# youssefg7/dl-sound-classification

Hardware: AMD Instinct MI355X
Metric: training clips/sec (EnvNet-v2, ESC-50 shape) (higher is better)
Workload: dtype bf16; 1 GPU; EnvNet-v2 train step (BC-mix, fwd, soft-CE, bwd, clip, Adam), ESC-50 shape; global_batch=256, per_gpu_batch=256, clip_samples=220500, parallelism=dp1, model=envnet_v2

## Files before the change

### dl-sound-classification_amd/csrc/gemm_common.h

```cpp
#pragma once
#include "common.h"
#include "optim_update.h"

namespace mgemm {

struct EpiDev {
  char* ptr;
  int dtype, act, accumulate, aux_dtype;
  int64_t ldc, rm_inner, rm_outer, rm_istride, rm_offset;
  const float* bias;
  const char* aux;
  int64_t ldaux;
  float alpha, act_scale;
  double* sqsum;
};

template <class R>
struct UpdateEpi {
  float* p;
  float* s0;
  float* s1;
  bf16* shadow;
  const float* coef;
  int64_t ld;
  int first;
  R rule;
};

struct DArgs {
  const bf16* a;
  const bf16* b;
  int64_t lda, ldb, M, N, K, kper;
  int split, nbm, nbn;
  int nfast;
  int gm;
  float* ws;
  EpiDev e;
  int mode;
  UpdateEpi<mopt::AdamRule> upd;
};

static __device__ __forceinline__ void epi_store(const EpiDev& e, int64_t m, int64_t n, float acc) {
  float v = acc * e.alpha;
  if (e.bias) v += e.bias[n];
  switch (e.act) {
    case MIA_ACT_RELU: v = fmaxf(v, 0.f); break;
    case MIA_ACT_GELU: v = gelu_erf(v); break;
    case MIA_DACT_NZ: {
      const float a = ld_elem(e.aux, e.aux_dtype, m * e.ldaux + n);
      v = a != 0.f ? v * e.act_scale : 0.f;
      break;
    }
    case MIA_DACT_GELU: v *= gelu_erf_grad(ld_elem(e.aux, e.aux_dtype, m * e.ldaux + n)); break;
    case MIA_ACT_ADD_AUX: v += ld_elem(e.aux, e.aux_dtype, m * e.ldaux + n); break;
    case MIA_ACT_GELU_SAVE:
      st_elem(const_cast<char*>(e.aux), e.aux_dtype, m * e.ldaux + n, v);
      v = gelu_erf(v);
      break;
    case MIA_ACT_GELU_SAVE_D:
      st_elem(const_cast<char*>(e.aux), e.aux_dtype, m * e.ldaux + n, gelu_erf_grad(v));
      v = gelu_erf(v);
      break;
    case MIA_DACT_MUL: v *= ld_elem(e.aux, e.aux_dtype, m * e.ldaux + n); break;
    default: break;
  }
  int64_t prow = m;
  if (e.rm_inner) {
    if (e.rm_offset == MIA_RM_DROP) {
      const int64_t x = m % e.rm_inner;
      if (x >= e.rm_outer) return;
      prow = (m / e.rm_inner) * e.rm_outer + x;
    } else {
      prow = (m / e.rm_inner) * e.rm_outer + (m % e.rm_inner) * e.rm_istride + e.rm_offset;
    }
  }
  const int64_t idx = prow * e.ldc + n;
  if (e.accumulate) v += ld_elem(e.ptr, e.dtype, idx);
  st_elem(e.ptr, e.dtype, idx, v);
}

static __device__ __forceinline__ void ld16(const void* p, int dtype, int64_t idx, float* f) {
  if (dtype == MIA_BF16) {
    const uint4* q = reinterpret_cast<const uint4*>(reinterpret_cast<const bf16*>(p) + idx);
#pragma unroll
    for (int h = 0; h < 2; ++h) {
      const uint4 u = q[h];
      const uint32_t w[4] = {u.x, u.y, u.z, u.w};
#pragma unroll
      for (int i = 0; i < 4; ++i) {
        f[8 * h + 2 * i] = __uint_as_float(w[i] << 16);
        f[8 * h + 2 * i + 1] = __uint_as_float(w[i] & 0xffff0000u);
      }
    }
  } else {
    const float4* q = reinterpret_cast<const float4*>(reinterpret_cast<const float*>(p) + idx);
#pragma unroll
    for (int h = 0; h < 4; ++h) {
      const float4 u = q[h];
      f[4 * h] = u.x; f[4 * h + 1] = u.y; f[4 * h + 2] = u.z; f[4 * h + 3] = u.w;
    }
  }
}

static __device__ __forceinline__ void st16(void* p, int dtype, int64_t idx, const float* o) {
  if (dtype == MIA_BF16) {
    uint32_t w[8];
#pragma unroll
    for (int c = 0; c < 8; ++c) {
      w[c] = pk_bf16(o[2 * c], o[2 * c + 1]);
    }
    uint4* d = reinterpret_cast<uint4*>(reinterpret_cast<bf16*>(p) + idx);
    d[0] = make_uint4(w[0], w[1], w[2], w[3]);
    d[1] = make_uint4(w[4], w[5], w[6], w[7]);
  } else {
    float4* d = reinterpret_cast<float4*>(reinterpret_cast<float*>(p) + idx);
#pragma unroll
    for (int q = 0; q < 4; ++q) d[q] = make_float4(o[4 * q], o[4 * q + 1], o[4 * q + 2], o[4 * q + 3]);
  }
}

static __device__ __forceinline__ void epi_store16(const EpiDev& e, int64_t m, int64_t n0, int64_t N, const float* v) {
  int64_t prow = m;
  if (e.rm_inner) {
    if (e.rm_offset == MIA_RM_DROP) {
      const int64_t x = m % e.rm_inner;
      if (x >= e.rm_outer) return;
      prow = (m / e.rm_inner) * e.rm_outer + x;
    } else {
      prow = (m / e.rm_inner) * e.rm_outer + (m % e.rm_inner) * e.rm_istride + e.rm_offset;
    }
  }
  const int64_t idx = prow * e.ldc + n0;
  const bool uses_aux = e.act == MIA_DACT_NZ || e.act == MIA_DACT_GELU || e.act == MIA_ACT_ADD_AUX ||
                        e.act == MIA_ACT_GELU_SAVE || e.act == MIA_ACT_GELU_SAVE_D || e.act == MIA_DACT_MUL;
  const int64_t aidx = m * e.ldaux + n0;
  const bool fast = n0 + 16 <= N && !e.accumulate &&
                    ((idx * (e.dtype == MIA_BF16 ? 2 : 4)) & 15) == 0 &&
                    ((reinterpret_cast<uintptr_t>(e.ptr)) & 15) == 0 &&
                    (!uses_aux || (((aidx * (e.aux_dtype == MIA_BF16 ? 2 : 4)) & 15) == 0 &&
                                   ((reinterpret_cast<uintptr_t>(e.aux)) & 15) == 0));
  if (!fast) {
    for (int c = 0; c < 16; ++c)
      if (n0 + c < N) epi_store(e, m, n0 + c, v[c]);
    return;
  }
  float o[16];
#pragma unroll
  for (int c = 0; c < 16; ++c) o[c] = v[c] * e.alpha;
  if (e.bias) {
    const float4* b4 = reinterpret_cast<const float4*>(e.bias + n0);
    const bool ba = ((reinterpret_cast<uintptr_t>(e.bias + n0)) & 15) == 0;
#pragma unroll
    for (int q = 0; q < 4; ++q) {
      float4 bb;
      if (ba) bb = b4[q];
      else bb = make_float4(e.bias[n0 + 4 * q], e.bias[n0 + 4 * q + 1], e.bias[n0 + 4 * q + 2], e.bias[n0 + 4 * q + 3]);
      o[4 * q] += bb.x; o[4 * q + 1] += bb.y; o[4 * q + 2] += bb.z; o[4 * q + 3] += bb.w;
    }
  }
  if (e.act == MIA_ACT_RELU) {
#pragma unroll
    for (int c = 0; c < 16; ++c) o[c] = fmaxf(o[c], 0.f);
  } else if (e.act == MIA_ACT_GELU) {
#pragma unroll
    for (int c = 0; c < 16; ++c) o[c] = gelu_erf(o[c]);
  } else if (e.act == MIA_ACT_GELU_SAVE) {
    st16(const_cast<char*>(e.aux), e.aux_dtype, aidx, o);
#pragma unroll
    for (int c = 0; c < 16; ++c) o[c] = gelu_erf(o[c]);
  } else if (e.act == MIA_ACT_GELU_SAVE_D) {
    float d[16];
#pragma unroll
    for (int c = 0; c < 16; ++c) d[c] = gelu_erf_grad(o[c]);
    st16(const_cast<char*>(e.aux), e.aux_dtype, aidx, d);
#pragma unroll
    for (int c = 0; c < 16; ++c) o[c] = gelu_erf(o[c]);
  } else if (uses_aux) {
    float a[16];
    ld16(e.aux, e.aux_dtype, aidx, a);
    if (e.act == MIA_DACT_NZ) {
#pragma unroll
      for (int c = 0; c < 16; ++c) o[c] = a[c] != 0.f ? o[c] * e.act_scale : 0.f;
    } else if (e.act == MIA_DACT_GELU) {
#pragma unroll
      for (int c = 0; c < 16; ++c) o[c] *= gelu_erf_grad(a[c]);
    } else if (e.act == MIA_DACT_MUL) {
#pragma unroll
      for (int c = 0; c < 16; ++c) o[c] *= a[c];
    } else {
#pragma unroll
      for (int c = 0; c < 16; ++c) o[c] += a[c];
    }
  }
  st16(e.ptr, e.dtype, idx, o);
}


EpiDev to_dev(const MiaEpilogue& e);
void launch_splitk_reduce(const float* ws, int split, int64_t M, int64_t N, const EpiDev& e, hipStream_t s);

int igemm_run(const MiaOperand& A, const MiaOperand& B, const MiaEpilogue& E, int64_t M, int64_t N, int64_t K,
              int compute, int split, void* workspace, hipStream_t s);
bool rowconv_ok(const MiaOperand& A, const MiaOperand& B, int64_t M, int64_t N, int64_t K, int compute, int split);
int rowconv_run(const MiaOperand& A, const MiaOperand& B, const MiaEpilogue& E, int64_t M, int64_t N, hipStream_t s);
bool rowwgrad_ok(const MiaOperand& A, const MiaOperand& B, int64_t M, int64_t N, int64_t K, int compute, int split);
int rowwgrad_run(const MiaOperand& A, const MiaOperand& B, const MiaEpilogue& E, int64_t M, int64_t N, int split,
                 void* workspace, hipStream_t s);
bool wgrad8_ok(const MiaOperand& A, const MiaOperand& B, int64_t M);
int wgrad8_run(const MiaOperand& A, const MiaOperand& B, const MiaEpilogue& E, int64_t M, int64_t N, int split,
               void* workspace, hipStream_t s);
bool tapwgrad_ok(const MiaOperand& A, const MiaOperand& B, int64_t M, int64_t N, int64_t K, int compute, int split);
int tapwgrad_run(const MiaOperand& A, const MiaOperand& B, const MiaEpilogue& E, int64_t M, int64_t N, int split,
                 void* workspace, hipStream_t s);
bool tapconv_ok(const MiaOperand& A, const MiaOperand& B, int64_t M, int64_t N, int64_t K, int compute, int split);
int tapconv_run(const MiaOperand& A, const MiaOperand& B, const MiaEpilogue& E, hipStream_t s);
bool dgemm_ok(const MiaOperand& A, const MiaOperand& B, int64_t M, int64_t N, int64_t K, int compute);
int dgemm_run(const MiaOperand& A, const MiaOperand& B, const MiaEpilogue& E, int64_t M, int64_t N, int64_t K,
              int split, void* workspace, hipStream_t s);
int tile_sqsum_run(const float* c, int64_t ldc, int64_t M, int64_t N, double* sqsum, hipStream_t s);
bool mg_ok(const MiaOperand& A, const MiaOperand& B, const MiaEpilogue& E, int64_t M, int64_t N, int64_t K,
           int compute);
int mg_split(int64_t M, int64_t N, int64_t K);
int64_t mg_workspace_bytes(int64_t M, int64_t N, int64_t K, int colsum, int a_colsum = 0);
int mg_run(const MiaOperand& A, const MiaOperand& B, const MiaEpilogue& E, int64_t M, int64_t N, int64_t K,
           void* workspace, hipStream_t s);


}
```

### dl-sound-classification_amd/csrc/wgrad8.hip

```cpp
#include "gemm_common.h"

namespace mgemm {

struct W8Args {
  const bf16* x;
  const bf16* dy;
  const float* ps;
  const float* pt;
  int n, h, w, oh, ow;
  int nblk;
  float* ws;
};

namespace {

constexpr int W8_NT = 512;
constexpr int W8_BP = 128;
constexpr int W8_WPX = W8_BP + 7;
constexpr int W8_XROW = W8_WPX * 64;
constexpr int W8_RING = 9;
constexpr int W8_DROW = W8_BP * 64;
constexpr int W8_XCH = (W8_WPX * 4 + W8_NT - 1) / W8_NT;

typedef short s16x8 __attribute__((ext_vector_type(8)));
typedef unsigned u32x4 __attribute__((ext_vector_type(4)));

__device__ __forceinline__ bf16x8 tr_frag(const char* p0, int stride) {
  const s16x4 lo = __builtin_amdgcn_ds_read_tr16_b64_v4i16((MIA_LDS s16x4*)(p0));
  const s16x4 hi = __builtin_amdgcn_ds_read_tr16_b64_v4i16((MIA_LDS s16x4*)(p0 + 4 * stride));
  const s16x8 c = {lo[0], lo[1], lo[2], lo[3], hi[0], hi[1], hi[2], hi[3]};
  return __builtin_bit_cast(bf16x8, c);
}

__device__ __forceinline__ u32x4 bn_relu_pack(u32x4 u, bool ok, const float* sc, const float* sh) {
  if (!ok) return u32x4{0u, 0u, 0u, 0u};
  uint32_t w4[4];
#pragma unroll
  for (int i = 0; i < 4; ++i) {
    const float lo = fmaxf(fmaf(__uint_as_float(u[i] << 16), sc[2 * i], sh[2 * i]), 0.f);
    const float hi = fmaxf(fmaf(__uint_as_float(u[i] & 0xffff0000u), sc[2 * i + 1], sh[2 * i + 1]), 0.f);
    w4[i] = pk_bf16(lo, hi);
  }
  return u32x4{w4[0], w4[1], w4[2], w4[3]};
}

__global__ __launch_bounds__(W8_NT) void wgrad8_kernel(W8Args g) {
  __shared__ __attribute__((aligned(16))) char smem[W8_RING * W8_XROW + 2 * W8_DROW];
  char* ring = smem;
  char* dys = smem + W8_RING * W8_XROW;
  const int t = threadIdx.x, lane = t & 63;
  const int ky = __builtin_amdgcn_readfirstlane(t >> 6);
  const int i16 = lane & 15, gq = lane >> 4;
  const int cg = t & 3;
  float sc[8], sh[8];
#pragma unroll
  for (int i = 0; i < 8; ++i) { sc[i] = g.ps[cg * 8 + i]; sh[i] = g.pt[cg * 8 + i]; }

  f32x16 acc[8];
#pragma unroll
  for (int q = 0; q < 8; ++q)
#pragma unroll
    for (int r = 0; r < 16; ++r) acc[q][r] = 0.f;

  const int nchunk = (g.ow + W8_BP - 1) / W8_BP;
  const int items = g.n * nchunk;
  u32x4 xr[W8_XCH], dr;
  uint32_t xok = 0;
  bool dok = false;
  const u32x4* xs = reinterpret_cast<const u32x4*>(g.x);
  const u32x4* ds = reinterpret_cast<const u32x4*>(g.dy);

  for (int item = blockIdx.x; item < items; item += gridDim.x) {
    const int b = item / nchunk;
    const int x0 = (item - b * nchunk) * W8_BP;
    auto load_x = [&](int iy) __attribute__((always_inline)) {
      xok = 0;
#pragma unroll
      for (int i = 0; i < W8_XCH; ++i) {
        const int q = t + W8_NT * i;
        const int px = x0 + (q >> 2);
        const bool ok = (q >> 2) < W8_WPX && px < g.w && iy < g.h;
        const int64_t off = ok ? ((((int64_t)b * g.h + iy) * g.w + px) * 4 + (q & 3)) : 0;
        xr[i] = xs[off];
        xok |= (uint32_t)ok << i;
      }
    };
    auto load_dy = [&](int oy) __attribute__((always_inline)) {
      const int px = x0 + (t >> 2);
      dok = oy >= 0 && oy < g.oh && px < g.ow;
      const int64_t off = dok ? ((((int64_t)b * g.oh + oy) * g.ow + px) * 4 + (t & 3)) : 0;
      dr = ds[off];
    };
    auto store_x = [&](int slot) __attribute__((always_inline)) {
#pragma unroll
      for (int i = 0; i < W8_XCH; ++i) {
        const int q = t + W8_NT * i;
        if ((q >> 2) < W8_WPX)
          *reinterpret_cast<u32x4*>(ring + slot * W8_XROW + q * 16) = bn_relu_pack(xr[i], (xok >> i) & 1u, sc, sh);
      }
    };
    auto store_dy = [&](int buf) __attribute__((always_inline)) {
      *reinterpret_cast<u32x4*>(dys + buf * W8_DROW + t * 16) = dok ? dr : u32x4{0u, 0u, 0u, 0u};
    };

    load_x(0);
    store_x(0);
    __syncthreads();
    for (int s = 0; s < g.h; ++s) {
      load_x(s + 1);
      load_dy(s - 6);
      const int oy = s - 7;
      if (oy >= 0) {
        const char* xrow = ring + ((oy + ky) % W8_RING) * W8_XROW;
        const char* drow = dys + (oy & 1) * W8_DROW;
#pragma unroll
        for (int ks = 0; ks < W8_BP / 16; ++ks) {
          const int kr = ks * 16 + 8 * (gq >> 1) + (i16 >> 2);
          const int c4 = 16 * (gq & 1) + 4 * (i16 & 3);
          const bf16x8 fa = tr_frag(drow + kr * 64 + c4 * 2, 64);
#pragma unroll
          for (int kx = 0; kx < 8; ++kx) {
            const bf16x8 fb = tr_frag(xrow + (kr + kx) * 64 + c4 * 2, 64);
            acc[kx] = __builtin_amdgcn_mfma_f32_32x32x16_bf16(fa, fb, acc[kx], 0, 0, 0);
          }
        }
      }
      if (s + 1 < g.h) store_x((s + 1) % W8_RING);
      if (s - 6 >= 0 && s - 6 < g.oh) store_dy((s - 6) & 1);
      __syncthreads();
    }
  }

  float* dst = g.ws + (int64_t)blockIdx.x * 32 * 2048 + ky * 256;
#pragma unroll
  for (int kx = 0; kx < 8; ++kx)
#pragma unroll
    for (int r = 0; r < 16; ++r) {
      const int co = (r & 3) + 8 * (r >> 2) + 4 * (lane >> 5);
      dst[(int64_t)co * 2048 + kx * 32 + (lane & 31)] = acc[kx][r];
    }
}

}

bool wgrad8_ok(const MiaOperand& A, const MiaOperand& B, int64_t M) {
  return A.dtype == MIA_BF16 && M == 32 && B.c == 32 && B.kh == 8 && B.kw == 8 && B.sw == 1 && B.ph == 0 &&
         B.pw == 0 && B.pre == MIA_PRE_AFFINE_RELU && B.h == B.oh + 7 && B.w == B.ow + 7;
}

int wgrad8_run(const MiaOperand& A, const MiaOperand& B, const MiaEpilogue& E, int64_t M, int64_t N, int split,
               void* workspace, hipStream_t s) {
  W8Args w8;
  w8.x = reinterpret_cast<const bf16*>(B.ptr);
  w8.dy = reinterpret_cast<const bf16*>(A.ptr);
  w8.ps = B.pre_scale; w8.pt = B.pre_shift;
  w8.n = B.n; w8.h = B.h; w8.w = B.w; w8.oh = B.oh; w8.ow = B.ow;
  const int64_t items = (int64_t)B.n * cdiv(B.ow, 128);
  w8.nblk = (int)std::min<int64_t>(std::min<int64_t>(split, 256), items);
  w8.ws = reinterpret_cast<float*>(workspace);
  wgrad8_kernel<<<w8.nblk, W8_NT, 0, s>>>(w8);
  hipError_t err = hipGetLastError();
  if (err != hipSuccess) return mia::fail(-(int)err, "wgrad8 launch: %s", hipGetErrorString(err));
  launch_splitk_reduce(w8.ws, w8.nblk, M, N, to_dev(E), s);
  MIA_LAUNCH_CHECK("splitk_reduce");
  return 0;
}

}
```

Before: 15510 clips/s.

## Pipeline wgrad8 kernel: shared transposed runs, interleaved staging, tail k-step skip

Reworks the 8x8 weight-gradient conv kernel. Each k-step now loads one transposed LDS run and derives all eight kx-shifted B fragments by register alignbit, replacing eight separate transposed reads. A and B fragments are double-buffered across k-steps, and the global loads and LDS stores for the next row are spread across specific k-steps with sched_group_barrier hints so they overlap the MFMAs. The kernel also preloads the first rows in batches and skips k-steps past the output width. The old path stays selectable through the MIA_WGRAD_V1 environment variable. The cost is more scheduling complexity and register pressure.

```diff
diff --git a/dl-sound-classification_amd/csrc/gemm_common.h b/dl-sound-classification_amd/csrc/gemm_common.h
--- a/dl-sound-classification_amd/csrc/gemm_common.h
+++ b/dl-sound-classification_amd/csrc/gemm_common.h
@@ -1,4 +1,6 @@
 #pragma once
+#include <cstdlib>
+
 #include "common.h"
 #include "optim_update.h"
 
@@ -195,6 +197,46 @@
   st16(e.ptr, e.dtype, idx, o);
 }
 
+
+static __device__ __forceinline__ bf16x8 tr_frag(const char* p0, int stride) {
+  typedef short s16x8_ __attribute__((ext_vector_type(8)));
+  const s16x4 lo = __builtin_amdgcn_ds_read_tr16_b64_v4i16((MIA_LDS s16x4*)(p0));
+  const s16x4 hi = __builtin_amdgcn_ds_read_tr16_b64_v4i16((MIA_LDS s16x4*)(p0 + 4 * stride));
+  const s16x8_ c = {lo[0], lo[1], lo[2], lo[3], hi[0], hi[1], hi[2], hi[3]};
+  return __builtin_bit_cast(bf16x8, c);
+}
+
+template <int G>
+struct TrRun {
+  uint32_t d[2 * G];
+};
+template <int G>
+static __device__ __forceinline__ TrRun<G> tr_run(const char* p0, int stride) {
+  typedef uint32_t u32x2_ __attribute__((ext_vector_type(2)));
+  TrRun<G> r;
+#pragma unroll
+  for (int q = 0; q < G; ++q) {
+    const u32x2_ v = __builtin_bit_cast(
+        u32x2_, __builtin_amdgcn_ds_read_tr16_b64_v4i16((MIA_LDS s16x4*)(p0 + 4 * q * stride)));
+    r.d[2 * q] = v[0];
+    r.d[2 * q + 1] = v[1];
+  }
+  return r;
+}
+template <int KX, int G>
+static __device__ __forceinline__ bf16x8 shifted_frag(const TrRun<G>& r) {
+  typedef uint32_t u32x4_ __attribute__((ext_vector_type(4)));
+  static_assert(KX >= 0 && (KX + 1) / 2 + 3 < 2 * G, "shift past the run");
+  u32x4_ o;
+#pragma unroll
+  for (int i = 0; i < 4; ++i) {
+    if constexpr (KX % 2 == 0) o[i] = r.d[KX / 2 + i];
+    else o[i] = __builtin_amdgcn_alignbit(r.d[KX / 2 + i + 1], r.d[KX / 2 + i], 16);
+  }
+  return __builtin_bit_cast(bf16x8, o);
+}
+
+static inline bool wgrad_v1() { const char* e = getenv("MIA_WGRAD_V1"); return e && e[0] == '1'; }
 
 EpiDev to_dev(const MiaEpilogue& e);
 void launch_splitk_reduce(const float* ws, int split, int64_t M, int64_t N, const EpiDev& e, hipStream_t s);
diff --git a/dl-sound-classification_amd/csrc/wgrad8.hip b/dl-sound-classification_amd/csrc/wgrad8.hip
--- a/dl-sound-classification_amd/csrc/wgrad8.hip
+++ b/dl-sound-classification_amd/csrc/wgrad8.hip
@@ -21,15 +21,20 @@
 constexpr int W8_RING = 9;
 constexpr int W8_DROW = W8_BP * 64;
 constexpr int W8_XCH = (W8_WPX * 4 + W8_NT - 1) / W8_NT;
-
-typedef short s16x8 __attribute__((ext_vector_type(8)));
+constexpr int W8_STAGE_KS = 5;
+static_assert(W8_XCH == 2 && W8_BP * 4 == W8_NT && W8_STAGE_KS + 2 < W8_BP / 16, "staging is spread over three k-steps");
+
 typedef unsigned u32x4 __attribute__((ext_vector_type(4)));
 
-__device__ __forceinline__ bf16x8 tr_frag(const char* p0, int stride) {
-  const s16x4 lo = __builtin_amdgcn_ds_read_tr16_b64_v4i16((MIA_LDS s16x4*)(p0));
-  const s16x4 hi = __builtin_amdgcn_ds_read_tr16_b64_v4i16((MIA_LDS s16x4*)(p0 + 4 * stride));
-  const s16x8 c = {lo[0], lo[1], lo[2], lo[3], hi[0], hi[1], hi[2], hi[3]};
-  return __builtin_bit_cast(bf16x8, c);
+__device__ __forceinline__ void mfma_taps(f32x16 (&acc)[8], bf16x8 fa, const TrRun<4>& run) {
+  acc[0] = __builtin_amdgcn_mfma_f32_32x32x16_bf16(fa, shifted_frag<0>(run), acc[0], 0, 0, 0);
+  acc[1] = __builtin_amdgcn_mfma_f32_32x32x16_bf16(fa, shifted_frag<1>(run), acc[1], 0, 0, 0);
+  acc[2] = __builtin_amdgcn_mfma_f32_32x32x16_bf16(fa, shifted_frag<2>(run), acc[2], 0, 0, 0);
+  acc[3] = __builtin_amdgcn_mfma_f32_32x32x16_bf16(fa, shifted_frag<3>(run), acc[3], 0, 0, 0);
+  acc[4] = __builtin_amdgcn_mfma_f32_32x32x16_bf16(fa, shifted_frag<4>(run), acc[4], 0, 0, 0);
+  acc[5] = __builtin_amdgcn_mfma_f32_32x32x16_bf16(fa, shifted_frag<5>(run), acc[5], 0, 0, 0);
+  acc[6] = __builtin_amdgcn_mfma_f32_32x32x16_bf16(fa, shifted_frag<6>(run), acc[6], 0, 0, 0);
+  acc[7] = __builtin_amdgcn_mfma_f32_32x32x16_bf16(fa, shifted_frag<7>(run), acc[7], 0, 0, 0);
 }
 
 __device__ __forceinline__ u32x4 bn_relu_pack(u32x4 u, bool ok, const float* sc, const float* sh) {
@@ -44,6 +49,18 @@
   return u32x4{w4[0], w4[1], w4[2], w4[3]};
 }
 
+__device__ __forceinline__ u32x4 bn_relu_pack_sel(u32x4 u, bool ok, const float* sc, const float* sh) {
+  u32x4 v;
+#pragma unroll
+  for (int i = 0; i < 4; ++i) {
+    const float lo = fmaxf(fmaf(__uint_as_float(u[i] << 16), sc[2 * i], sh[2 * i]), 0.f);
+    const float hi = fmaxf(fmaf(__uint_as_float(u[i] & 0xffff0000u), sc[2 * i + 1], sh[2 * i + 1]), 0.f);
+    v[i] = ok ? pk_bf16(lo, hi) : 0u;
+  }
+  return v;
+}
+
+template <bool V1>
 __global__ __launch_bounds__(W8_NT) void wgrad8_kernel(W8Args g) {
   __shared__ __attribute__((aligned(16))) char smem[W8_RING * W8_XROW + 2 * W8_DROW];
   char* ring = smem;
@@ -73,6 +90,7 @@
   for (int item = blockIdx.x; item < items; item += gridDim.x) {
     const int b = item / nchunk;
     const int x0 = (item - b * nchunk) * W8_BP;
+    const int nks = V1 ? W8_BP / 16 : min(W8_BP / 16, (g.ow - x0 + 15) >> 4);
     auto load_x = [&](int iy) __attribute__((always_inline)) {
       xok = 0;
 #pragma unroll
@@ -99,34 +117,108 @@
           *reinterpret_cast<u32x4*>(ring + slot * W8_XROW + q * 16) = bn_relu_pack(xr[i], (xok >> i) & 1u, sc, sh);
       }
     };
+    auto store_x0 = [&](int slot) __attribute__((always_inline)) {
+      *reinterpret_cast<u32x4*>(ring + slot * W8_XROW + t * 16) = bn_relu_pack_sel(xr[0], xok & 1u, sc, sh);
+    };
+    auto store_x1 = [&](int slot) __attribute__((always_inline)) {
+      if (ky == 0 && (t >> 2) < W8_WPX - W8_BP)
+        *reinterpret_cast<u32x4*>(ring + slot * W8_XROW + (t + W8_NT) * 16) = bn_relu_pack(xr[1], (xok >> 1) & 1u, sc, sh);
+    };
     auto store_dy = [&](int buf) __attribute__((always_inline)) {
       *reinterpret_cast<u32x4*>(dys + buf * W8_DROW + t * 16) = dok ? dr : u32x4{0u, 0u, 0u, 0u};
     };
 
-    load_x(0);
-    store_x(0);
+    int s0 = 0;
+    if constexpr (V1) {
+      load_x(0);
+      store_x(0);
+    } else {
+      load_dy(0);
+#pragma unroll
+      for (int r0 = 0; r0 < 8; r0 += 4) {
+        u32x4 pr[4][W8_XCH];
+        uint32_t pok[4];
+#pragma unroll
+        for (int r = 0; r < 4; ++r) {
+          load_x(r0 + r);
+          pok[r] = xok;
+#pragma unroll
+          for (int i = 0; i < W8_XCH; ++i) pr[r][i] = xr[i];
+        }
+#pragma unroll
+        for (int r = 0; r < 4; ++r) {
+          xok = pok[r];
+#pragma unroll
+          for (int i = 0; i < W8_XCH; ++i) xr[i] = pr[r][i];
+          store_x(r0 + r);
+        }
+      }
+      store_dy(0);
+      s0 = 7;
+    }
     __syncthreads();
-    for (int s = 0; s < g.h; ++s) {
-      load_x(s + 1);
-      load_dy(s - 6);
+    for (int s = s0; s < g.h; ++s) {
+      if constexpr (V1) {
+        load_x(s + 1);
+        load_dy(s - 6);
+      }
       const int oy = s - 7;
       if (oy >= 0) {
         const char* xrow = ring + ((oy + ky) % W8_RING) * W8_XROW;
         const char* drow = dys + (oy & 1) * W8_DROW;
-#pragma unroll
-        for (int ks = 0; ks < W8_BP / 16; ++ks) {
-          const int kr = ks * 16 + 8 * (gq >> 1) + (i16 >> 2);
-          const int c4 = 16 * (gq & 1) + 4 * (i16 & 3);
-          const bf16x8 fa = tr_frag(drow + kr * 64 + c4 * 2, 64);
-#pragma unroll
-          for (int kx = 0; kx < 8; ++kx) {
-            const bf16x8 fb = tr_frag(xrow + (kr + kx) * 64 + c4 * 2, 64);
-            acc[kx] = __builtin_amdgcn_mfma_f32_32x32x16_bf16(fa, fb, acc[kx], 0, 0, 0);
+        if constexpr (V1) {
+#pragma unroll
+          for (int ks = 0; ks < W8_BP / 16; ++ks) {
+            const int kr = ks * 16 + 8 * (gq >> 1) + (i16 >> 2);
+            const int c4 = 16 * (gq & 1) + 4 * (i16 & 3);
+            const bf16x8 fa = tr_frag(drow + kr * 64 + c4 * 2, 64);
+#pragma unroll
+            for (int kx = 0; kx < 8; ++kx) {
+              const bf16x8 fb = tr_frag(xrow + (kr + kx) * 64 + c4 * 2, 64);
+              acc[kx] = __builtin_amdgcn_mfma_f32_32x32x16_bf16(fa, fb, acc[kx], 0, 0, 0);
+            }
+          }
+        } else {
+          const int fo = (8 * (gq >> 1) + (i16 >> 2)) * 64 + (16 * (gq & 1) + 4 * (i16 & 3)) * 2;
+          bf16x8 fa[2];
+          TrRun<4> run[2];
+          fa[0] = tr_frag(drow + fo, 64);
+          run[0] = tr_run<4>(xrow + fo, 64);
+          load_x(s + 1);
+          load_dy(s - 6);
+#pragma unroll
+          for (int ks = 0; ks < W8_BP / 16; ++ks) {
+            if (ks >= nks) break;
+            const int c = ks & 1;
+            if (ks == W8_STAGE_KS + 2) store_x1((s + 1) % W8_RING);
+            if (ks + 1 < W8_BP / 16) {
+              fa[c ^ 1] = tr_frag(drow + fo + (ks + 1) * 1024, 64);
+              run[c ^ 1] = tr_run<4>(xrow + fo + (ks + 1) * 1024, 64);
+            }
+            mfma_taps(acc, fa[c], run[c]);
+            if (ks == W8_STAGE_KS) store_x0((s + 1) % W8_RING);
+            if (ks == W8_STAGE_KS + 1) store_dy((s - 6) & 1);
+            if (ks + 1 < W8_BP / 16) {
+#pragma unroll
+              for (int q = 0; q < 6; ++q) {
+                __builtin_amdgcn_sched_group_barrier(0x008, 1, 0);
+                __builtin_amdgcn_sched_group_barrier(0x100, 1, 0);
+              }
+              __builtin_amdgcn_sched_group_barrier(0x008, 2, 0);
+            } else {
+              __builtin_amdgcn_sched_group_barrier(0x008, 8, 0);
+            }
           }
         }
       }
-      if (s + 1 < g.h) store_x((s + 1) % W8_RING);
-      if (s - 6 >= 0 && s - 6 < g.oh) store_dy((s - 6) & 1);
+      if constexpr (V1) {
+        if (s + 1 < g.h) store_x((s + 1) % W8_RING);
+        if (s - 6 >= 0 && s - 6 < g.oh) store_dy((s - 6) & 1);
+      } else {
+        if (nks <= W8_STAGE_KS) store_x0((s + 1) % W8_RING);
+        if (nks <= W8_STAGE_KS + 1) store_dy((s - 6) & 1);
+        if (nks <= W8_STAGE_KS + 2) store_x1((s + 1) % W8_RING);
+      }
       __syncthreads();
     }
   }
@@ -158,7 +250,8 @@
   const int64_t items = (int64_t)B.n * cdiv(B.ow, 128);
   w8.nblk = (int)std::min<int64_t>(std::min<int64_t>(split, 256), items);
   w8.ws = reinterpret_cast<float*>(workspace);
-  wgrad8_kernel<<<w8.nblk, W8_NT, 0, s>>>(w8);
+  if (wgrad_v1()) wgrad8_kernel<true><<<w8.nblk, W8_NT, 0, s>>>(w8);
+  else wgrad8_kernel<false><<<w8.nblk, W8_NT, 0, s>>>(w8);
   hipError_t err = hipGetLastError();
   if (err != hipSuccess) return mia::fail(-(int)err, "wgrad8 launch: %s", hipGetErrorString(err));
   launch_splitk_reduce(w8.ws, w8.nblk, M, N, to_dev(E), s);
```

New measurement: 15590 clips/s (median of 6 runs). Within noise of the previous version (+0.5%).
